# chenhuims/DistributedDeepLearningSpark

Hardware: AMD Instinct MI355X
Metric: images/sec (whole node) ResNet-50 ImageNet-shape at 1/2/4/8 MI355X (higher is better)
Workload: dtype bf16; 1 GPU; model=resnet50, global_batch=256, image=224, per_gpu_batch=256, parallelism=dp1, optimizer=sgd-momentum, buckets=4

## Files before the change

distributeddeeplearningspark_amd/csrc/include/ddl_ops.h:

```cpp
#pragma once
#include <hip/hip_runtime.h>
#include <stdint.h>

namespace ddl {

inline uint32_t drop_t8(double p) {
  if (!(p > 0.0)) return 0u;
  const double t = p * 256.0 + 0.5;
  return t < 1.0 ? 1u : (t >= 255.0 ? 255u : (uint32_t)t);
}
inline float drop_scale8(uint32_t t8) { return t8 ? (float)(256.0 / (256.0 - (double)t8)) : 1.f; }

constexpr int kBnShards = 32;
constexpr int kMaxPartials = 512;

int bn_partial_rows(long M, int C);
int splitk_finalize(float* ws, void* y, const float* bias, float* stats, long M, int C, int relu, int splits,
                    long slab_stride, hipStream_t s, long brows = 0,
                    long zbias = 0);
int bn_stats(const void* x, float* ws, long M, int C, hipStream_t s);
int bn_finalize(const float* ws, int S, long M, int C, const float* gamma, const float* beta, float eps,
                float momentum, float* running_mean, float* running_var, float* save_mean, float* save_invstd,
                float* scale, float* shift, hipStream_t s);
int bn_apply(const void* x, const float* scale, const float* shift, const void* resid, void* y, void* mask, long M,
             int C, int relu, hipStream_t s, const float* res_scale = nullptr, const float* res_shift = nullptr);
int bn_bwd_reduce(const void* dy, const void* x, const void* y, const float* scale, const float* shift,
                  const float* mean, float* ws, long M, int C, int mode, hipStream_t s);
int bn_bwd_finalize(const float* ws, int S, long M, int C, const float* gamma, const float* mean, const float* invstd,
                    float* dgamma, float* dbeta, float* coef, hipStream_t s);
int bn_bwd_dx(const void* dy, const void* x, const void* y, const float* scale, const float* shift,
              const float* coef, void* dx, void* dres, long M, int C, int mode, hipStream_t s,
              const void* x2 = nullptr, const float* mean2 = nullptr, float* ws2 = nullptr);

int bn_fold_sums(const void* w, long ldw, const float* P, const float* wsg, const float* mean, const float* wsy,
                 int rows, float* sums, float* s, int Co, int Ci, hipStream_t st);
int bn_fold_coef(const void* w, long ldw, const float* P, const float* S, const float* s, const float* coef, void* WA,
                 void* WAt, void* Gm, float* kv, float* dW, long lddw, int Co, int Ci, hipStream_t st);
int bn_fold_kv(const void* WA, const void* Gm, const float* sg, const float* s, long M, float* kv, int Co, int Ci,
               hipStream_t st);
int gram_colsum(const void* y2, long ld, long M, int Ci, float* S, float* s, int cus, hipStream_t st);
int bn_fold_fwd_stats(const void* w, long ldw, const float* S, const float* s, long M, float* ws, int Co, int Ci,
                      hipStream_t st);

bool pool3s2_bn_bwd_ok(int N, int H, int W, int C, int Ho, int Wo, int k = 3);
int pool3s2_bn_bwd(const void* dy, const uint8_t* am, const void* x, const float* scale, const float* shift,
                   const float* mean, const float* coef, float* ws, int S, void* dx, int N, int H, int W, int C, int Ho,
                   int Wo, hipStream_t s, int k = 3);

int maxpool_fwd(const void* x, void* y, uint8_t* argmax, int N, int H, int W, int C, int Ho, int Wo, int kh, int kw,
                int sh, int sw, int ph, int pw, hipStream_t s, const float* scale = nullptr, const float* shift = nullptr);
int maxpool_bwd(const void* dy, const uint8_t* argmax, void* dx, int N, int H, int W, int C, int Ho, int Wo, int kh,
                int kw, int sh, int sw, int ph, int pw, hipStream_t s);
int avgpool_global_fwd(const void* x, void* y, int N, int HW, int C, hipStream_t s);
int avgpool_global_bwd(const void* dy, void* dx, int N, int HW, int C, hipStream_t s);

int softmax_xent(const void* logits, int logits_bf16, const int64_t* labels, const float* target_probs,
                 float* loss_rows, void* dlogits, int B, int K, long ld, float grad_scale, float label_smoothing,
                 int ignore_index, hipStream_t s, const float* grad_scale_dev = nullptr, float* loss_out = nullptr,
                 float out_scale = 1.f, int zrows = 0);
int label_count_inv(const int64_t* labels, long n, int ignore_index, float* inv, hipStream_t s);
int rows_sum_scaled(const float* rows, long n, float scale, const float* dev, float* out, hipStream_t s);
int scale_bf16_dev(void* x, long n, const float* s_dev, hipStream_t s);
int mse_fwd_bwd(const float* pred, const float* target, long n, float* loss, float* grad, hipStream_t s);
int prob_xent(const float* p, const int64_t* labels, const float* target, float* loss_rows, float* dp, int B, int K,
              float eps, float scale, int ignore_index, hipStream_t s);
int mask_count_inv(const uint8_t* mask, long n, float* inv, hipStream_t s);
int temporal_xent(const float* logits, const int64_t* labels, const float* target_probs, const uint8_t* mask,
                  const float* inv_dev, float inv_host, float* loss_rows, float* dlogits, long R, int K, hipStream_t s);
int temporal_reg(const float* pred, const float* target, const uint8_t* mask, long R, int F, int mae, float* loss,
                 float* grad, hipStream_t s);

int cast_f32_bf16(const float* x, void* y, long n, hipStream_t s);
int cast_bf16_f32(const void* x, float* y, long n, hipStream_t s);
int sum_rows_bf16(const void* x, void* y, int R, long n, hipStream_t s);
int relu_bwd(const void* dy, const void* y, void* dx, long n, hipStream_t s);
// ... 224 lines not shown
```

distributeddeeplearningspark_amd/csrc/kernels/gemm_stream.hip:

```cpp
#include "ddl_gemm_kernel.h"

namespace ddl {
namespace gst {

constexpr int THREADS = 256;
constexpr int BM = 64;
constexpr int LDS_BUDGET = 80 * 1024;
typedef __attribute__((address_space(3))) void lds_t;

template <int WN, int K, bool CSM = false>
struct Cfg {
  static constexpr int NB = 4 * WN;
  static constexpr int RN = WN / 16;
  static constexpr int KS = K / 32;
  static constexpr int CPR = K / 8;
  static constexpr int TILE = BM * K * 2;
  static constexpr int D = TILE / 1024 / 4;
  static constexpr int OCPR = NB / 8;
  static constexpr int STAGE = BM * NB * 2;
  static constexpr int RPP = THREADS / OCPR;
  static constexpr int S = BM / RPP;
  static constexpr int SV = CSM ? 2 * S : S;
  static constexpr int NBUF_FIT = (LDS_BUDGET - STAGE) / TILE;
  static constexpr int NBUF = NBUF_FIT > 4 ? 4 : NBUF_FIT;
  static constexpr int LDS = NBUF * TILE + STAGE;
  static_assert(NBUF >= 2, "A ring needs two buffers");
  static_assert(D >= 1 && OCPR >= 8 && RPP >= 1 && BM % RPP == 0, "shape");
  static_assert((NBUF - 1) * (D + SV) <= 63, "vmcnt range");
  static_assert(4 * 2 * OCPR * 8 * 4 <= STAGE, "stats reduction fits in the staging buffer");
};

template <int CPR>
__device__ __forceinline__ int sw(int r) {
  if constexpr (CPR == 8) return (r >> 1) & 7;
  else return r & 15;
}

template <int N>
__device__ __forceinline__ void wait_vm() {
  __builtin_amdgcn_s_waitcnt((N & 15) | ((N >> 4) << 14) | 0x0F70);
}

template <class CF, int SV = CF::S>
__device__ __forceinline__ void wait_tile(int younger_store_tiles) {
  constexpr int base = (CF::NBUF - 1) * CF::D;
  switch (younger_store_tiles) {
    case 0: wait_vm<base>(); break;
    case 1: wait_vm<base + SV>(); break;
    case 2: wait_vm<base + 2 * SV>(); break;
    default: wait_vm<base + 3 * SV>(); break;
  }
}

template <class CF, bool DUAL = false>
__device__ __forceinline__ void stage_a(const bf16_t* __restrict__ A, long lda, int M, int m0, char* slot, int w,
                                        int lane, const bf16_t* __restrict__ A2 = nullptr, long lda2 = 0) {
#pragma unroll
  for (int i = 0; i < CF::D; ++i) {
    const int blk = i * 4 + w;
    const int u = blk * 64 + lane;
    const int r = u / CF::CPR, cp = u % CF::CPR;
    const int c = cp ^ sw<CF::CPR>(r);
    const int gr = min(m0 + r, M - 1);
    const bf16_t* src = A + (long)gr * lda + c * 8;
    if constexpr (DUAL) {
      if (c >= CF::CPR / 2) src = A2 + (long)gr * lda2 + (c - CF::CPR / 2) * 8;
    }
    const uint32_t dst = __builtin_amdgcn_readfirstlane((uint32_t) reinterpret_cast<uintptr_t>((lds_t*)(slot + blk * 1024)));
    asm volatile("s_mov_b32 m0, %1\n\tglobal_load_lds_dwordx4 %0, off" ::"v"(src), "s"(dst) : "memory", "m0");
  }
}

}

typedef __attribute__((ext_vector_type(2))) unsigned u32x2_t;
typedef __attribute__((ext_vector_type(4))) unsigned u32x4_t;
__device__ __forceinline__ u32x4_t ald128(const void* p) {
  u32x4_t v;
  asm volatile("global_load_dwordx4 %0, %1, off" : "=v"(v) : "v"(p) : "memory");
  return v;
}
__device__ __forceinline__ u32x2_t ald64(const void* p) {
  u32x2_t v;
  asm volatile("global_load_dwordx2 %0, %1, off" : "=v"(v) : "v"(p) : "memory");
  return v;
}
__device__ __forceinline__ unsigned ald32(const void* p) {
  unsigned v;
  asm volatile("global_load_dword %0, %1, off" : "=v"(v) : "v"(p) : "memory");
  return v;
}
__device__ __forceinline__ unsigned ald16(const void* p) {
  unsigned v;
  asm volatile("global_load_ushort %0, %1, off" : "=v"(v) : "v"(p) : "memory");
  return v;
}
__device__ __forceinline__ unsigned ald8(const void* p) {
  unsigned v;
  asm volatile("global_load_ubyte %0, %1, off" : "=v"(v) : "v"(p) : "memory");
  return v;
}
template <bool ASM> __device__ __forceinline__ u32x4_t sld128(const void* p) {
// ... 378 lines not shown
    (void)hipGetDevice(&dev);
    if (hipDeviceGetAttribute(&cus, hipDeviceAttributeMultiprocessorCount, dev) != hipSuccess || cus <= 0) cus = 256;
  }
  return cus;
}

template <int WN, int K, int BMODE>
int launch_ws(const GemmParams& p, hipStream_t s) {
  using CF = gst::Cfg<WN, K>;
  constexpr bool kRes = !(WN == 64 && K == 128);
  constexpr bool kBnr = CF::NB <= (K >= 256 ? 64 : 128);
  const int panels = p.N / CF::NB;
  const int mt = (p.M + gst::BM - 1) / gst::BM;
  const int gx = std::max(1, std::min(mt, 2 * num_cus() / std::max(1, panels)));
  if (p.colscale || p.relu_mask_out) {
    constexpr bool kCsm = BMODE == OP_KC && ((WN == 64 && K == 64) || (WN == 32 && K == 128) || (WN == 32 && K == 256));
    if constexpr (kCsm) {
      if (!p.colscale || !p.resid || p.bnr_x || p.bnr_premask || p.stats || p.rsub_h) return (int)hipErrorInvalidValue;
      hipLaunchKernelGGL((gemm_stream_kernel<WN, K, BMODE, true, 0, true>), dim3(gx, panels), dim3(gst::THREADS), 0, s, p);
    } else {
      return (int)hipErrorInvalidValue;
    }
  } else if (p.bnr_premask) {
    if constexpr (kBnr && kRes && BMODE == OP_RC) {
      if (!p.bnr_mask || p.bnr_scale) return (int)hipErrorInvalidValue;
      if (p.resid)
        hipLaunchKernelGGL((gemm_stream_kernel<WN, K, BMODE, true, 3>), dim3(gx, panels), dim3(gst::THREADS), 0, s, p);
      else
        hipLaunchKernelGGL((gemm_stream_kernel<WN, K, BMODE, false, 3>), dim3(gx, panels), dim3(gst::THREADS), 0, s, p);
    } else {
      return (int)hipErrorInvalidValue;
    }
  } else if (p.bnr_x && p.bnr_scale) {
    constexpr bool kRes2 = WN == 16 && K == 256 && BMODE == OP_RC;
    if constexpr (kBnr) {
      if (p.resid) {
        if constexpr (kRes2)
          hipLaunchKernelGGL((gemm_stream_kernel<WN, K, BMODE, true, 2>), dim3(gx, panels), dim3(gst::THREADS), 0, s, p);
        else
          return (int)hipErrorInvalidValue;
      } else {
        hipLaunchKernelGGL((gemm_stream_kernel<WN, K, BMODE, false, 2>), dim3(gx, panels), dim3(gst::THREADS), 0, s, p);
      }
    } else {
      return (int)hipErrorInvalidValue;
    }
  } else if (p.bnr_x) {
    if constexpr (kBnr && kRes) {
      if (p.resid)
        hipLaunchKernelGGL((gemm_stream_kernel<WN, K, BMODE, true, 1>), dim3(gx, panels), dim3(gst::THREADS), 0, s, p);
      else
        hipLaunchKernelGGL((gemm_stream_kernel<WN, K, BMODE, false, 1>), dim3(gx, panels), dim3(gst::THREADS), 0, s, p);
    } else if constexpr (kBnr) {
      if (p.resid) return (int)hipErrorInvalidValue;
      hipLaunchKernelGGL((gemm_stream_kernel<WN, K, BMODE, false, 1>), dim3(gx, panels), dim3(gst::THREADS), 0, s, p);
    } else {
      return (int)hipErrorInvalidValue;
    }
  } else if (p.resid) {
    if constexpr (kRes)
      hipLaunchKernelGGL((gemm_stream_kernel<WN, K, BMODE, true>), dim3(gx, panels), dim3(gst::THREADS), 0, s, p);
    else
      return (int)hipErrorInvalidValue;
  } else {
    hipLaunchKernelGGL((gemm_stream_kernel<WN, K, BMODE, false>), dim3(gx, panels), dim3(gst::THREADS), 0, s, p);
  }
  return (int)hipGetLastError();
// ... 73 lines not shown
```

distributeddeeplearningspark_amd/csrc/ops_bindings.cpp:

```cpp
#include <torch/extension.h>
#include <ATen/hip/impl/HIPStreamMasqueradingAsCUDA.h>
#include <ATen/DeviceGuard.h>

#include "ddl_ops.h"

namespace py = pybind11;
using namespace ddl;

namespace {

inline hipStream_t cur_stream() { return at::hip::getCurrentHIPStreamMasqueradingAsCUDA().stream(); }

#define CK(cond, ...) TORCH_CHECK(cond, __VA_ARGS__)
#define GPU(x) CK((x).is_cuda(), #x " must be a GPU tensor")
#define BF16(x) CK((x).scalar_type() == at::kBFloat16 && (x).is_contiguous(), #x " must be contiguous bf16")
#define F32(x) CK((x).scalar_type() == at::kFloat && (x).is_contiguous(), #x " must be contiguous fp32")
#define HIP_OK(expr)                                                                  \
  do {                                                                                \
    int _e = (expr);                                                                  \
    CK(_e == 0, "HIP launch failed: ", hipGetErrorString((hipError_t)_e)); \
  } while (0)

template <class T>
T* optr(const c10::optional<at::Tensor>& t) {
// ... 95 lines not shown
void bn_fold_sums_(const at::Tensor& w, const at::Tensor& P, const at::Tensor& wsg, const at::Tensor& mean,
                   c10::optional<at::Tensor> wsy, const at::Tensor& sums, const at::Tensor& s) {
  GPU(w); F32(P); F32(wsg); F32(mean); F32(sums); F32(s);
  CK(w.scalar_type() == at::kBFloat16 && w.dim() == 2 && w.stride(1) == 1, "bn_fold_sums: w [Co, Ci] bf16");
  const int64_t Co = w.size(0), Ci = w.size(1);
  CK(P.numel() == Co * Ci && wsg.numel() == (int64_t)kBnShards * 2 * Co && mean.numel() >= Co && sums.numel() == 2 * Co &&
         s.numel() == Ci,
     "bn_fold_sums: shapes");
  if (wsy) { F32(*wsy); CK(wsy->numel() % (2 * Ci) == 0 && wsy->numel() > 0, "bn_fold_sums: wsy [rows, 2, Ci]"); }
  at::DeviceGuard g(w.device());
  HIP_OK(bn_fold_sums(w.data_ptr(), w.stride(0), P.data_ptr<float>(), wsg.data_ptr<float>(), mean.data_ptr<float>(),
                      optr<const float>(wsy), wsy ? (int)(wsy->numel() / (2 * Ci)) : 0, sums.data_ptr<float>(),
                      s.data_ptr<float>(), (int)Co, (int)Ci, cur_stream()));
}

void gram_colsum_(const at::Tensor& y2, const at::Tensor& S, const at::Tensor& s) {
  GPU(y2); GPU(S); GPU(s); F32(S); F32(s);
  CK(y2.scalar_type() == at::kBFloat16 && y2.dim() == 2 && y2.stride(1) == 1 && y2.stride(0) % 8 == 0 &&
         ((uintptr_t)y2.data_ptr() % 16) == 0,
     "gram_colsum: y2 [M, Ci] bf16, 16-B aligned rows");
  const int64_t M = y2.size(0), Ci = y2.size(1);
  CK((Ci == 64 || Ci == 128 || Ci == 256) && M > 0 && y2.stride(0) >= Ci, "gram_colsum: Ci in {64, 128, 256}");
  CK(S.numel() == Ci * Ci && s.numel() == Ci && ((uintptr_t)S.data_ptr() % 16) == 0, "gram_colsum: S [Ci, Ci], s [Ci]");
  CK(S.device() == y2.device() && s.device() == y2.device(), "gram_colsum: y2, S and s on one device");
  at::DeviceGuard g(y2.device());
  static int cus_of[64] = {};
  const int dev = y2.device().index();
  int cus = dev >= 0 && dev < 64 ? cus_of[dev] : 0;
  if (!cus) {
    if (hipDeviceGetAttribute(&cus, hipDeviceAttributeMultiprocessorCount, dev) != hipSuccess || cus <= 0) cus = 256;
    if (dev >= 0 && dev < 64) cus_of[dev] = cus;
  }
  HIP_OK(gram_colsum(y2.data_ptr(), y2.stride(0), M, (int)Ci, S.data_ptr<float>(), s.data_ptr<float>(), cus, cur_stream()));
}

void bn_fold_fwd_stats_(const at::Tensor& w, const at::Tensor& S, const at::Tensor& s, int64_t M, const at::Tensor& ws) {
  GPU(w); GPU(S); GPU(s); GPU(ws); F32(S); F32(s); F32(ws);
  CK(S.device() == w.device() && s.device() == w.device() && ws.device() == w.device(),
     "bn_fold_fwd_stats: w, S, s and ws on one device");
  CK(w.scalar_type() == at::kBFloat16 && w.dim() == 2 && w.stride(1) == 1, "bn_fold_fwd_stats: w [Co, Ci] bf16");
  const int64_t Co = w.size(0), Ci = w.size(1);
  CK(Ci % 32 == 0 && Ci <= 256 && M > 0 && S.numel() == Ci * Ci && s.numel() == Ci && ws.numel() >= 2 * Co &&
         ((uintptr_t)S.data_ptr() % 16) == 0,
     "bn_fold_fwd_stats: Ci % 32 == 0, Ci <= 256, S [Ci, Ci], s [Ci], ws [>= 1, 2, Co]");
  at::DeviceGuard g(w.device());
  HIP_OK(bn_fold_fwd_stats(w.data_ptr(), w.stride(0), S.data_ptr<float>(), s.data_ptr<float>(), M, ws.data_ptr<float>(),
                           (int)Co, (int)Ci, cur_stream()));
}

void bn_fold_coef_(const at::Tensor& w, const at::Tensor& P, const at::Tensor& S, const at::Tensor& s,
                   const at::Tensor& coef, const at::Tensor& WA, const at::Tensor& WAt, const at::Tensor& Gm,
                   const at::Tensor& kv, const at::Tensor& dW) {
  GPU(w); F32(P); F32(S); F32(s); F32(coef); BF16(WA); BF16(WAt); BF16(Gm); F32(kv);
  CK(w.scalar_type() == at::kBFloat16 && w.dim() == 2 && w.stride(1) == 1, "bn_fold_coef: w [Co, Ci] bf16");
  const int64_t Co = w.size(0), Ci = w.size(1);
  CK(Co % 128 == 0 && Ci % 64 == 0, "bn_fold_coef: Co % 128, Ci % 64");
  CK(P.numel() == Co * Ci && S.numel() == Ci * Ci && s.numel() == Ci && coef.numel() >= 3 * Co && WA.numel() == Co * Ci &&
         WAt.numel() == Co * Ci && Gm.numel() == Ci * Ci && kv.numel() == Ci,
     "bn_fold_coef: shapes");
  CK(dW.is_cuda() && dW.scalar_type() == at::kFloat && dW.dim() == 2 && dW.size(0) == Co && dW.size(1) == Ci &&
         dW.stride(1) == 1 && dW.stride(0) >= Ci,
     "bn_fold_coef: dW [Co, Ci] fp32");
  at::DeviceGuard g(w.device());
  HIP_OK(bn_fold_coef(w.data_ptr(), w.stride(0), P.data_ptr<float>(), S.data_ptr<float>(), s.data_ptr<float>(),
                      coef.data_ptr<float>(), WA.data_ptr(), WAt.data_ptr(), Gm.data_ptr(), kv.data_ptr<float>(),
                      dW.data_ptr<float>(), dW.stride(0), (int)Co, (int)Ci, cur_stream()));
// ... 586 lines not shown
  OPT_CHECK(w, g);
  F32(acc);
  CK(acc.numel() == w.numel(), "rmsprop: state size");
  if (w16) BF16(*w16);
  at::DeviceGuard gd(w.device());
  HIP_OK(rmsprop_step(w.data_ptr<float>(), g.data_ptr<float>(), acc.data_ptr<float>(), optr<void>(w16), w.numel(),
                      (float)lr, (float)rho, (float)eps, (float)wd, (float)gscale, cur_stream()));
}
void sumsq_(const at::Tensor& x, const at::Tensor& out) {
  GPU(x); F32(x); F32(out);
  CK(x.numel() % 4 == 0, "sumsq: multiple of 4");
  at::DeviceGuard gd(x.device());
  HIP_OK(sumsq_f32(x.data_ptr<float>(), x.numel(), out.data_ptr<float>(), cur_stream()));
}

}

void register_ops(py::module& m) {
  m.attr("BN_SHARDS") = (int)kBnShards;
  m.def("bn_stats", &bn_stats_);
  m.def("splitk_finalize", &splitk_finalize_, py::arg("ws"), py::arg("y"), py::arg("C"), py::arg("bias"), py::arg("relu"),
        py::arg("stats"), py::arg("splits") = 0, py::arg("brows") = 0, py::arg("zbias") = 0);
  m.def("bn_partial_rows", &bn_partial_rows_);
  m.def("bn_finalize", &bn_finalize_);
  m.def("bn_apply", &bn_apply_, py::arg("x"), py::arg("scale"), py::arg("shift"), py::arg("resid"), py::arg("y"),
        py::arg("C"), py::arg("relu"), py::arg("mask") = py::none(), py::arg("res_scale") = py::none(),
        py::arg("res_shift") = py::none());
  m.def("bn_bwd_reduce", &bn_bwd_reduce_);
  m.def("bn_bwd_finalize", &bn_bwd_finalize_);
  m.def("bn_fold_sums", &bn_fold_sums_);
  m.def("bn_fold_coef", &bn_fold_coef_);
  m.def("bn_fold_kv", &bn_fold_kv_);
  m.def("gram_colsum", &gram_colsum_);
  m.def("bn_fold_fwd_stats", &bn_fold_fwd_stats_);
  m.def("bn_bwd_dx", &bn_bwd_dx_);
  m.def("bn_bwd_dx_red", &bn_bwd_dx_red_);
  m.def("pool3s2_bn_bwd", &pool3s2_bn_bwd_, py::arg("dy"), py::arg("am"), py::arg("x"), py::arg("scale"),
        py::arg("shift"), py::arg("mean"), py::arg("coef_or_ws"), py::arg("dx"), py::arg("k") = 3);
  m.def("pool3s2_bn_bwd_ok", [](int64_t N, int64_t H, int64_t W, int64_t C, int64_t Ho, int64_t Wo, int64_t k) {
    return pool3s2_bn_bwd_ok((int)N, (int)H, (int)W, (int)C, (int)Ho, (int)Wo, (int)k);
  });
  m.def("maxpool_fwd", &maxpool_fwd_, "NHWC max pool (byte argmax); optional fused BN affine + ReLU on load",
        py::arg("x"), py::arg("y"), py::arg("am"), py::arg("kh"), py::arg("kw"), py::arg("sh"), py::arg("sw"),
        py::arg("ph"), py::arg("pw"), py::arg("scale") = py::none(), py::arg("shift") = py::none());
  m.def("maxpool_bwd", &maxpool_bwd_);
  m.def("avgpool_fwd", &avgpool_fwd_);
  m.def("avgpool_bwd", &avgpool_bwd_);
  m.def("softmax_xent", &softmax_xent_, "fused softmax cross-entropy", py::arg("logits"), py::arg("labels"),
        py::arg("probs"), py::arg("loss_rows"), py::arg("dlogits"), py::arg("grad_scale"), py::arg("smoothing"),
        py::arg("ignore_index"), py::arg("grad_scale_dev") = py::none(), py::arg("loss_out") = py::none(),
        py::arg("out_scale") = 1.0, py::arg("zrows") = 0);
  m.def("label_count_inv", &label_count_inv_);
  m.def("rows_sum_scaled", &rows_sum_scaled_);
  m.def("pad_cols_bf16", &pad_cols_bf16_, "zero-padded copy of a row-strided bf16 view");
  m.def("zero_ranges", &zero_ranges_, "zero up to 8 contiguous device buffers in one launch", py::arg("buffers"));
  m.def("gather_bf16", &gather_bf16_, "out[i] = src[idx[i]] (0 where idx < 0)", py::arg("src"), py::arg("idx"),
        py::arg("out"), py::arg("src_extent"));
  m.def("scatter_add_f32", &scatter_add_f32_, "dst[idx[i]] += src[i] (idx injective, < 0 skipped)", py::arg("src"),
        py::arg("idx"), py::arg("dst"), py::arg("dst_extent"));
  m.def("scale_bf16_dev", &scale_bf16_dev_);
  m.def("cast_f32_bf16", &cast_f32_bf16_);
  m.def("sum_rows_bf16", &sum_rows_bf16_);
  m.def("cast_bf16_f32", &cast_bf16_f32_);
  m.def("relu_bwd", &relu_bwd_);
  m.def("add_bf16", &add_bf16_);
  m.def("bias_grad", &bias_grad_, py::arg("dy"), py::arg("db"), py::arg("N"), py::arg("accumulate"),
// ... 34 lines not shown
```

distributeddeeplearningspark_amd/ops/fused_blocks.py:

```python
from __future__ import annotations

import weakref

import torch

from . import conv as CV
from . import determinism as _det
from . import gemm as G
from . import zpad as ZP
from ._native import C
from .norm import new_stats_workspace, partials_workspace, pool_epoch
from .streams import on_grad_stream


class _ConvBNState:

    __slots__ = ("g", "yc", "y", "mean", "invstd", "scale", "shift", "mode", "mask", "pre_reduced", "fold", "gram",
                 "__weakref__")

    def __init__(self):
        self.pre_reduced = None
        self.fold = False
        self.gram = None

# ... 321 lines not shown
    ps = new_stats_workspace(-(-(Ci * Ci + Ci) // 64), dev).view(-1)
    S, s = ps[: Ci * Ci].view(Ci, Ci), ps[Ci * Ci : Ci * Ci + Ci]
    C().gram_colsum(xm, S, s)
    stats = new_stats_workspace(Co, dev)
    C().bn_fold_fwd_stats(conv.kernel.data.view(Co, Ci), S, s, M, stats)
    gamma = None if bn.gamma is None else bn.gamma.master
    beta = None if bn.beta is None else bn.beta.master
    rm, rv = bn._states["moving_mean"], bn._states["moving_variance"]
    st = _ConvBNState()
    st.g, st.yc, st.y, st.mask = g, None, None, None
    st.scale, st.shift, st.mean, st.invstd = torch.empty(4, Co, dtype=torch.float32, device=dev).unbind(0)
    C().bn_finalize(stats, M, Co, gamma, beta, bn.epsilon, 1.0 - bn.momentum, rm, rv, st.mean, st.invstd, st.scale,
                    st.shift)
    st.gram = (S, s, pool_epoch(dev))
    return st


def _fold_down_forward(block, x, y2, g3, gd):
    M, Co = g3.M, g3.Co
    if tuple(y2.shape) != (g3.N, g3.H, g3.W, g3.Ci):
        raise RuntimeError("folding projection block: conv2's output does not match conv3's geometry")
    y2 = y2.contiguous()
    s3 = _fold_fwd_stats(block.c3, y2.view(M, g3.Ci), g3)
    sd = _fold_fwd_stats(block.down, x.view(M, gd.Ci), gd)
    s3.mask = torch.empty(-(-M * Co // 32) * 4, dtype=torch.uint8, device=x.device)
    y = torch.empty((g3.N, g3.H, g3.W, Co), dtype=torch.bfloat16, device=x.device)
    G.linear_dual_fwd(y2.view(M, g3.Ci), block.c3.conv.kernel.data.view(Co, g3.Ci), s3.scale,
                      x.view(M, gd.Ci), block.down.conv.kernel.data.view(Co, gd.Ci), sd.scale,
                      shift1=s3.shift, shift2=sd.shift, relu=True, out=y.view(M, Co), relu_mask_out=s3.mask)
    s3.y, s3.mode, sd.mode = y, 3, 0
    return sd, s3


def fold_conv_bn_backward(w, gw, g2, y2, ws_g, mean, invstd, gamma, dgamma, dbeta, bnr2=None, out=None, gram=None,
                          need_dx=True, exact_colsum=False):
    M, Co = g2.shape
    Ci = y2.shape[1]
    dev = g2.device
    if gram is not None:
        S, s = gram
        P = new_stats_workspace(-(-(Co * Ci) // 64), dev).view(-1)[: Co * Ci].view(Co, Ci)
        G.linear_wgrad(g2, y2, P)
        wsy = None
    else:
        ps = new_stats_workspace(-(-(Co * Ci + Ci * Ci + Ci) // 64), dev).view(-1)
        P, S = ps[: Co * Ci].view(Co, Ci), ps[Co * Ci : Co * Ci + Ci * Ci].view(Ci, Ci)
        s = ps[Co * Ci + Ci * Ci : Co * Ci + Ci * Ci + Ci]
        G.linear_wgrad(g2, y2, P)
        G.linear_wgrad(y2, y2, S)
        wsy = partials_workspace(M, Ci, dev)
        C().bn_stats(y2, wsy, Ci)
    f32 = torch.empty(5 * Co + Ci, dtype=torch.float32, device=dev)
    sums, coef, kv = f32[: 2 * Co], f32[2 * Co : 5 * Co], f32[5 * Co :]
    C().bn_fold_sums(w, P, ws_g, mean, wsy, sums, s)
    C().bn_bwd_finalize(sums, M, Co, gamma, mean, invstd, dgamma, dbeta, coef)
    b16 = torch.empty(2 * Co * Ci + Ci * Ci, dtype=torch.bfloat16, device=dev)
    WA, WAt, Gm = b16[: Co * Ci].view(Co, Ci), b16[Co * Ci : 2 * Co * Ci].view(Ci, Co), b16[2 * Co * Ci :].view(Ci, Ci)
    C().bn_fold_coef(w, P, S, s, coef, WA, WAt, Gm, kv, gw)
    if not need_dx:
        return None, sums.view(2, Co)
    if exact_colsum:
        C().bn_fold_kv(WA, Gm, sums[:Co], s, M, kv)
    r = G.linear_fwd(y2, Gm, bias=kv)
    if out is None:
        out = torch.empty((M, Ci), dtype=torch.bfloat16, device=dev)
    G.linear_dgrad(g2, WA, out=out, resid=r, bnr=bnr2, wt=WAt)
    return out, sums.view(2, Co)


def _fold_bn3_backward(unit, s3, s2, g, ws_g, bnr2):
    return _fold_unit_backward(unit, s3, s2.y, g, ws_g, bnr2)


def _fold_unit_backward(unit, st, xin, g, ws_g, bnr2, need_dx=True, exact_colsum=False):
    conv, bn = unit.conv, unit.bn
    geo = st.g
    M, Co, Ci = geo.M, geo.Co, geo.Ci
    dx = torch.empty((geo.N, geo.H, geo.W, Ci), dtype=torch.bfloat16, device=g.device) if need_dx else None
    gram = None
    if st.gram is not None and st.gram[2] == pool_epoch(g.device):
        gram = st.gram[:2]
    fold_conv_bn_backward(conv.kernel.data.view(Co, Ci), conv.kernel.grad.view(Co, Ci), g.view(M, Co), xin.view(M, Ci),
                          ws_g, st.mean, st.invstd, bn.gamma.master, bn.gamma.grad,
                          None if bn.beta is None else bn.beta.grad, bnr2=bnr2,
                          out=None if dx is None else dx.view(M, Ci), gram=gram, need_dx=need_dx,
                          exact_colsum=exact_colsum)
    if bn.grad_hook is not None:
        bn.grad_hook()
    if conv.grad_hook is not None:
        conv.grad_hook()
    return dx


def _same_tensor(a, b) -> bool:
    return (a.data_ptr() == b.data_ptr() and a.shape == b.shape and a.stride() == b.stride()
            and a._version == b._version)


# ... 292 lines not shown
```

distributeddeeplearningspark_amd/ops/gemm.py:

```python
from __future__ import annotations

import math

import torch

from . import determinism as _det
from ._native import C

KC, RC, KC_GATHER, RC_GATHER, RC_TAPS, KC_GATHER8, RC_GATHER8 = 0, 1, 2, 3, 4, 5, 6
EPI_BF16, EPI_F32, EPI_F32_ATOMIC = 0, 1, 2
TILE256 = 4
TILE_STREAM = 5
TILE_CONV3 = 6
_TILES = {0: (128, 128), 1: (128, 64), 2: (64, 128), 3: (64, 64), TILE256: (256, 256), TILE_STREAM: (64, 256),
          TILE_CONV3: (224, 128)}
_ONE_PER_CU = (TILE256,)
_CU = 256
import os as _os

_USE256 = "auto"


_USE_STREAM = "1"
_TILE_FILL = 2.0
# ... 237 lines not shown
            r = gemm(dy, w, ws, M, K, N, KC, RC, dy.stride(0), w.stride(0), K, EPI_F32, tile=3,
                     k_split=math.ceil(N / splits / 64) * 64, defer_slabs=True)
        if isinstance(r, tuple):
            C().splitk_finalize(r[0], out, K, None, False, stats, r[1])
        else:
            C().splitk_finalize(ws, out, K, None, False, stats)
        return out
    if M >= _WT_MIN_M and not use_stream(M, K, N, KC, RC, EPI_BF16, dy.stride(0), out.stride(0), aux=gelu_pre,
                                         relu=act, resid=resid, ldr=ldr):
        wt = transpose(w) if wt is None else wt
        fb = _bnr_plain_ok(bnr, stats, resid, gelu_pre, K)
        gemm(dy, wt, out, M, K, N, KC, KC, dy.stride(0), wt.stride(0), out.stride(0), EPI_BF16, resid=resid,
             ldr=ldr, relu=act, aux=gelu_pre, stats=stats, resid_mask=resid_mask, rsub=rsub, bnr=bnr if fb else None)
        if fb:
            bnr["done"] = True
        return out
    if (bnr is not None and stats is None
            and ("scale" not in bnr or (resid is None and rsub is None) or (rsub is None and (K, N) == (64, 256)))
            and use_stream(M, K, N, KC, RC, EPI_BF16, dy.stride(0), out.stride(0), aux=gelu_pre, relu=act,
                           resid=resid, ldr=ldr)):
        gemm(dy, w, out, M, K, N, KC, RC, dy.stride(0), w.stride(0), out.stride(0), EPI_BF16, resid=resid, ldr=ldr,
             relu=act, aux=gelu_pre, resid_mask=resid_mask, tile=TILE_STREAM, bnr=bnr, rsub=rsub)
        bnr["done"] = True
        return out
    fb = _bnr_plain_ok(bnr, stats, resid, gelu_pre, K) and not use_stream(
        M, K, N, KC, RC, EPI_BF16, dy.stride(0), out.stride(0), aux=gelu_pre, relu=act, resid=resid, ldr=ldr)
    gemm(dy, w, out, M, K, N, KC, RC, dy.stride(0), w.stride(0), out.stride(0), EPI_BF16, resid=resid,
         ldr=ldr, relu=act, aux=gelu_pre, stats=stats, resid_mask=resid_mask, rsub=rsub, bnr=bnr if fb else None)
    if fb:
        bnr["done"] = True
    return out


def _bnr_plain_ok(bnr, stats, resid, gelu_pre, ncols) -> bool:
    return (bnr is not None and stats is None and gelu_pre is None and ncols % 8 == 0
            and (bnr["x"].is_contiguous() if bnr.get("x") is not None else bool(bnr.get("premask")))
            and (resid is None or (resid.stride(0) % 4 == 0 and resid.data_ptr() % 8 == 0)))


def transpose(w):
    R, Cc = w.shape
    if w.stride(1) != 1 or R % 8 or Cc % 8 or w.stride(0) % 8:
        return w.t().contiguous()
    if w.is_contiguous():
        from . import derived

        return derived.taps_transpose(w, (0,), (Cc, R))
    out = torch.empty((Cc, R), dtype=w.dtype, device=w.device)
    C().transpose_bf16(w, out)
    return out


def linear_wgrad(dy, x2, gw):
    M, N = dy.shape
    K = x2.shape[1]
    rounds = None if (big_wgrad(N, K, M) and _SPLITK_SLABS_MODE == "auto") else _LINEAR_WGRAD_ROUNDS
    return gemm(dy, x2, gw, N, K, M, RC, RC, dy.stride(0), x2.stride(0), gw.stride(0), EPI_F32, beta=1.0,
                split_rounds=rounds)


def matmul(a, b, trans_a=False, trans_b=False, out=None, alpha=1.0):
    M = a.shape[1] if trans_a else a.shape[0]
    K = a.shape[0] if trans_a else a.shape[1]
    N = b.shape[0] if trans_b else b.shape[1]
    if out is None:
        out = torch.empty((M, N), dtype=torch.bfloat16, device=a.device)
# ... 4 lines not shown
```

Before: 13410 images/sec.

## Fuse fold-BN backward wgrad and dgrad into a single pass over g and y2

Adds a HIP kernel for the Co=256/Ci=64 folded conv+BN backward. It streams g and y2 through LDS once, computing the P = g^T·y2 weight-gradient product and the t = g·(gamma*invstd*W) data-gradient product together. A second GEMM pass then adds y2·Gm+kv using t as the residual, replacing the separate linear_wgrad, linear_fwd and linear_dgrad launches. This cuts re-reads of the large g activation, but adds a bf16 intermediate t, atomics into P, and one-off weight scaling per block.

```diff
diff --git a/distributeddeeplearningspark_amd/csrc/include/ddl_gemm_stream.h b/distributeddeeplearningspark_amd/csrc/include/ddl_gemm_stream.h
--- /dev/null
+++ b/distributeddeeplearningspark_amd/csrc/include/ddl_gemm_stream.h
@@ -0,0 +1,28 @@
+#pragma once
+#include "ddl_common.h"
+
+namespace ddl {
+namespace gst {
+
+constexpr int THREADS = 256;
+constexpr int BM = 64;
+typedef __attribute__((address_space(3))) void lds_t;
+
+template <int CPR>
+__device__ __forceinline__ int sw(int r) {
+  if constexpr (CPR == 8) return (r >> 1) & 7;
+  else return r & 15;
+}
+
+template <int N>
+__device__ __forceinline__ void wait_vm() {
+  __builtin_amdgcn_s_waitcnt((N & 15) | ((N >> 4) << 14) | 0x0F70);
+}
+
+__device__ __forceinline__ void dma_1k(const void* src, char* dst_block) {
+  const uint32_t dst = __builtin_amdgcn_readfirstlane((uint32_t) reinterpret_cast<uintptr_t>((lds_t*)dst_block));
+  asm volatile("s_mov_b32 m0, %1\n\tglobal_load_lds_dwordx4 %0, off" ::"v"(src), "s"(dst) : "memory", "m0");
+}
+
+}
+}
diff --git a/distributeddeeplearningspark_amd/csrc/include/ddl_ops.h b/distributeddeeplearningspark_amd/csrc/include/ddl_ops.h
--- a/distributeddeeplearningspark_amd/csrc/include/ddl_ops.h
+++ b/distributeddeeplearningspark_amd/csrc/include/ddl_ops.h
@@ -41,6 +41,9 @@
 int gram_colsum(const void* y2, long ld, long M, int Ci, float* S, float* s, int cus, hipStream_t st);
 int bn_fold_fwd_stats(const void* w, long ldw, const float* S, const float* s, long M, float* ws, int Co, int Ci,
                       hipStream_t st);
+int fold_bwd_pass1(const void* g, long ldg, const void* y2, long ldy, const void* w, long ldw, const float* gamma,
+                   const float* invstd, long M, int Co, int Ci, float* P, void* t, long ldt, void* wa_out,
+                   int workgroups, hipStream_t st);
 
 bool pool3s2_bn_bwd_ok(int N, int H, int W, int C, int Ho, int Wo, int k = 3);
 int pool3s2_bn_bwd(const void* dy, const uint8_t* am, const void* x, const float* scale, const float* shift,
diff --git a/distributeddeeplearningspark_amd/csrc/kernels/fold_bwd.hip b/distributeddeeplearningspark_amd/csrc/kernels/fold_bwd.hip
--- /dev/null
+++ b/distributeddeeplearningspark_amd/csrc/kernels/fold_bwd.hip
@@ -0,0 +1,238 @@
+#include "ddl_gemm_stream.h"
+#include "ddl_ops.h"
+
+namespace ddl {
+namespace fbw {
+
+using gst::BM;
+using gst::sw;
+using gst::wait_vm;
+
+constexpr int THREADS = 256;
+constexpr int CO = 256, CI = 64;
+constexpr int GROW = CO * 2, YROW = CI * 2;
+constexpr int GT = BM * GROW, YT = BM * YROW;
+constexpr int GCPR = CO / 8, YCPR = CI / 8;
+constexpr int NBUF = 3;
+constexpr int CHAIN = 8;
+constexpr int MIN_TILES = 16;
+constexpr int STAGE = BM * CI * 2;
+constexpr int S = STAGE / 16 / THREADS;
+
+struct Cfg {
+  static constexpr int SLOT = GT + YT;
+  static constexpr int D = SLOT / 1024 / 4;
+  static constexpr int LDS = NBUF * SLOT + STAGE;
+  static_assert((NBUF - 1) * (D + S) <= 63, "vmcnt range");
+  static_assert(LDS <= 160 * 1024, "LDS");
+};
+
+__device__ __forceinline__ void stage(const bf16_t* __restrict__ g, long ldg, const bf16_t* __restrict__ y, long ldy,
+                                      int M, int m0, char* slot, int w, int lane) {
+#pragma unroll
+  for (int i = 0; i < Cfg::D; ++i) {
+    const int blk = i * 4 + w;
+    const bf16_t* src;
+    if (i < GT / 4096) {
+      const int u = blk * 64 + lane;
+      const int r = u / GCPR, c = (u % GCPR) ^ sw<GCPR>(r);
+      src = g + (long)min(m0 + r, M - 1) * ldg + c * 8;
+    } else {
+      const int u = (blk - GT / 1024) * 64 + lane;
+      const int r = u / YCPR, c = (u % YCPR) ^ sw<YCPR>(r);
+      src = y + (long)min(m0 + r, M - 1) * ldy + c * 8;
+    }
+    gst::dma_1k(src, slot + blk * 1024);
+  }
+}
+
+template <int CPR>
+__device__ __forceinline__ bf16x8 tr_frag(const char* lds, int kk, int c0, int lane) {
+  const int g = lane >> 4, li = lane & 15, q = li >> 2, p = li & 3;
+  const int k1 = kk * 32 + 8 * g + q, k2 = k1 + 4;
+  const int col = c0 + 4 * p;
+  const int ch = col >> 3, within = (col & 7) * 2;
+  const int o1 = k1 * (CPR * 16) + ((ch ^ sw<CPR>(k1)) << 4) + within;
+  const int o2 = k2 * (CPR * 16) + ((ch ^ sw<CPR>(k2)) << 4) + within;
+  const s16x4 lo = __builtin_amdgcn_ds_read_tr16_b64_v4i16((DDL_LDS s16x4*)(lds + o1));
+  const s16x4 hi = __builtin_amdgcn_ds_read_tr16_b64_v4i16((DDL_LDS s16x4*)(lds + o2));
+  const s16x8 r = {lo[0], lo[1], lo[2], lo[3], hi[0], hi[1], hi[2], hi[3]};
+  return __builtin_bit_cast(bf16x8, r);
+}
+
+__device__ __forceinline__ void wait_tile(int younger_store_tiles) {
+  constexpr int base = (NBUF - 1) * Cfg::D;
+  switch (younger_store_tiles) {
+    case 0: wait_vm<base>(); break;
+    case 1: wait_vm<base + S>(); break;
+    default: wait_vm<base + 2 * S>(); break;
+  }
+}
+
+}
+
+__global__ __launch_bounds__(fbw::THREADS, 1) void fold_bwd_pass1_kernel(
+    const bf16_t* __restrict__ g, long ldg, const bf16_t* __restrict__ y2, long ldy, const bf16_t* __restrict__ wgt,
+    long ldw, const float* __restrict__ gamma, const float* __restrict__ invstd, int M, float* __restrict__ P,
+    bf16_t* __restrict__ t, long ldt, bf16_t* __restrict__ wa_out) {
+  using namespace fbw;
+  using CF = Cfg;
+  __shared__ __attribute__((aligned(16))) char smem[CF::LDS];
+  char* const stg = smem + NBUF * CF::SLOT;
+  const int lane = threadIdx.x & 63, w = threadIdx.x >> 6;
+  const int mh = w >> 1, nh = w & 1;
+  const int mt = (M + BM - 1) / BM;
+  const int nloc = ((int)blockIdx.x < mt) ? (mt - 1 - (int)blockIdx.x) / (int)gridDim.x + 1 : 0;
+
+  bf16x8 wa[2][CO / 32];
+#pragma unroll
+  for (int rn = 0; rn < 2; ++rn)
+#pragma unroll
+    for (int ks = 0; ks < CO / 32; ++ks) {
+      const int ci = 32 * nh + 16 * rn + (lane & 15);
+      s16x8 v;
+#pragma unroll
+      for (int j = 0; j < 8; ++j) {
+        const int co = 32 * ks + 8 * (lane >> 4) + j;
+        const float a = gamma[co] * invstd[co];
+        const bf16_t b = f2bf(a * bf2f(wgt[(long)co * ldw + ci]));
+        v[j] = (short)b;
+      }
+      wa[rn][ks] = __builtin_bit_cast(bf16x8, v);
+    }
+  if (wa_out && blockIdx.x == 0) {
+    for (int u = threadIdx.x; u < CO * CI; u += THREADS) {
+      const int co = u / CI, ci = u % CI;
+      const float a = gamma[co] * invstd[co];
+      wa_out[u] = f2bf(a * bf2f(wgt[(long)co * ldw + ci]));
+    }
+  }
+  wait_vm<0>();
+  auto tile_m0 = [&](int i) { return min((int)blockIdx.x + i * (int)gridDim.x, mt - 1) * BM; };
+
+#pragma unroll
+  for (int s = 0; s < NBUF - 1; ++s) stage(g, ldg, y2, ldy, M, tile_m0(s), smem + s * CF::SLOT, w, lane);
+
+  f32x4 acc[4][4], tot[4][4];
+#pragma unroll
+  for (int cb = 0; cb < 4; ++cb)
+#pragma unroll
+    for (int nb = 0; nb < 4; ++nb)
+      acc[cb][nb] = tot[cb][nb] = f32x4{0.f, 0.f, 0.f, 0.f};
+  auto fold_chain = [&]() {
+#pragma unroll
+    for (int cb = 0; cb < 4; ++cb)
+#pragma unroll
+      for (int nb = 0; nb < 4; ++nb) {
+        tot[cb][nb] += acc[cb][nb];
+        acc[cb][nb] = f32x4{0.f, 0.f, 0.f, 0.f};
+      }
+  };
+  const int oc = threadIdx.x % YCPR, orow = threadIdx.x / YCPR;
+  constexpr int RPP = THREADS / YCPR;
+
+  for (int i = 0; i < nloc; ++i) {
+    const int m0 = tile_m0(i);
+    const int ahead = i + NBUF - 1;
+    stage(g, ldg, y2, ldy, M, tile_m0(ahead), smem + (ahead % NBUF) * CF::SLOT, w, lane);
+    wait_tile(min(i, NBUF - 1));
+    __builtin_amdgcn_s_barrier();
+    char* const gbuf = smem + (i % NBUF) * CF::SLOT;
+    char* const ybuf = gbuf + GT;
+    if (m0 + BM > M) {
+      const int rz = M - m0;
+      for (int u = threadIdx.x; u < (BM - rz) * YCPR; u += THREADS)
+        *reinterpret_cast<uint4*>(ybuf + rz * YROW + u * 16) = make_uint4(0u, 0u, 0u, 0u);
+      __builtin_amdgcn_s_waitcnt(0xC07F);
+      __builtin_amdgcn_s_barrier();
+    }
+
+    f32x4 tacc[2][2];
+#pragma unroll
+    for (int mb = 0; mb < 2; ++mb)
+#pragma unroll
+      for (int rn = 0; rn < 2; ++rn) tacc[mb][rn] = f32x4{0.f, 0.f, 0.f, 0.f};
+#pragma unroll
+    for (int ks = 0; ks < CO / 32; ++ks)
+#pragma unroll
+      for (int mb = 0; mb < 2; ++mb) {
+        const int r = 32 * mh + 16 * mb + (lane & 15);
+        const int c = 4 * ks + (lane >> 4);
+        const bf16x8 a = *reinterpret_cast<const bf16x8*>(gbuf + r * GROW + ((c ^ sw<GCPR>(r)) << 4));
+#pragma unroll
+        for (int rn = 0; rn < 2; ++rn) tacc[mb][rn] = mfma16x16x32(wa[rn][ks], a, tacc[mb][rn]);
+      }
+
+    __builtin_amdgcn_sched_barrier(0);
+    {
+      bf16x8 gf[4][2];
+#pragma unroll
+      for (int cb = 0; cb < 4; ++cb)
+#pragma unroll
+        for (int kk = 0; kk < 2; ++kk) gf[cb][kk] = tr_frag<GCPR>(gbuf, kk, 64 * w + 16 * cb, lane);
+#pragma unroll
+      for (int nb = 0; nb < 4; ++nb) {
+        const bf16x8 y0 = tr_frag<YCPR>(ybuf, 0, 16 * nb, lane);
+        const bf16x8 y1 = tr_frag<YCPR>(ybuf, 1, 16 * nb, lane);
+#pragma unroll
+        for (int cb = 0; cb < 4; ++cb) {
+          acc[cb][nb] = mfma16x16x32(gf[cb][0], y0, acc[cb][nb]);
+          acc[cb][nb] = mfma16x16x32(gf[cb][1], y1, acc[cb][nb]);
+        }
+        __builtin_amdgcn_sched_barrier(0);
+      }
+    }
+    if (i % CHAIN == CHAIN - 1) fold_chain();
+
+#pragma unroll
+    for (int mb = 0; mb < 2; ++mb) {
+      const int r = 32 * mh + 16 * mb + (lane & 15);
+#pragma unroll
+      for (int rn = 0; rn < 2; ++rn) {
+        const int nl = 32 * nh + 16 * rn + 4 * (lane >> 4);
+        *reinterpret_cast<uint2*>(stg + r * YROW + (((nl >> 3) ^ sw<YCPR>(r)) << 4) + (nl & 7) * 2) =
+            make_uint2(pack_bf16x2(tacc[mb][rn][0], tacc[mb][rn][1]), pack_bf16x2(tacc[mb][rn][2], tacc[mb][rn][3]));
+      }
+    }
+    __builtin_amdgcn_s_waitcnt(0xC07F);
+    __builtin_amdgcn_s_barrier();
+
+#pragma unroll
+    for (int ps = 0; ps < S; ++ps) {
+      const int r = orow + ps * RPP;
+      const uint4 v = *reinterpret_cast<const uint4*>(stg + r * YROW + ((oc ^ sw<YCPR>(r)) << 4));
+      if (m0 + r < M) *reinterpret_cast<uint4*>(t + (long)(m0 + r) * ldt + oc * 8) = v;
+    }
+  }
+  wait_vm<0>();
+
+  fold_chain();
+  if (nloc > 0) {
+#pragma unroll
+    for (int cb = 0; cb < 4; ++cb)
+#pragma unroll
+      for (int nb = 0; nb < 4; ++nb)
+#pragma unroll
+        for (int e = 0; e < 4; ++e) {
+          const long idx = (long)(64 * w + 16 * cb + 4 * (lane >> 4) + e) * CI + 16 * nb + (lane & 15);
+          atomicAdd(P + idx, tot[cb][nb][e]);
+        }
+  }
+}
+
+int fold_bwd_pass1(const void* g, long ldg, const void* y2, long ldy, const void* w, long ldw, const float* gamma,
+                   const float* invstd, long M, int Co, int Ci, float* P, void* t, long ldt, void* wa_out,
+                   int workgroups, hipStream_t st) {
+  auto al16 = [](const void* q) { return (uintptr_t)q % 16 == 0; };
+  if (Co != fbw::CO || Ci != fbw::CI || M <= 0 || M >= (1L << 30) || workgroups <= 0 || !g || !y2 || !w || !gamma ||
+      !invstd || !P || !t || ldg % 8 || ldy % 8 || ldt % 8 || ldg < Co || ldy < Ci || ldt < Ci || ldw < Ci || !al16(g) ||
+      !al16(y2) || !al16(t))
+    return (int)hipErrorInvalidValue;
+  const int mt = (int)((M + gst::BM - 1) / gst::BM);
+  const dim3 grid((unsigned)std::max(1, std::min((mt + fbw::MIN_TILES - 1) / fbw::MIN_TILES, workgroups)));
+  hipLaunchKernelGGL(fold_bwd_pass1_kernel, grid, dim3(fbw::THREADS), 0, st, (const bf16_t*)g, ldg, (const bf16_t*)y2,
+                     ldy, (const bf16_t*)w, ldw, gamma, invstd, (int)M, P, (bf16_t*)t, ldt, (bf16_t*)wa_out);
+  return (int)hipGetLastError();
+}
+
+}
diff --git a/distributeddeeplearningspark_amd/csrc/kernels/gemm_stream.hip b/distributeddeeplearningspark_amd/csrc/kernels/gemm_stream.hip
--- a/distributeddeeplearningspark_amd/csrc/kernels/gemm_stream.hip
+++ b/distributeddeeplearningspark_amd/csrc/kernels/gemm_stream.hip
@@ -1,12 +1,10 @@
 #include "ddl_gemm_kernel.h"
+#include "ddl_gemm_stream.h"
 
 namespace ddl {
 namespace gst {
 
-constexpr int THREADS = 256;
-constexpr int BM = 64;
 constexpr int LDS_BUDGET = 80 * 1024;
-typedef __attribute__((address_space(3))) void lds_t;
 
 template <int WN, int K, bool CSM = false>
 struct Cfg {
@@ -30,17 +28,6 @@
   static_assert(4 * 2 * OCPR * 8 * 4 <= STAGE, "stats reduction fits in the staging buffer");
 };
 
-template <int CPR>
-__device__ __forceinline__ int sw(int r) {
-  if constexpr (CPR == 8) return (r >> 1) & 7;
-  else return r & 15;
-}
-
-template <int N>
-__device__ __forceinline__ void wait_vm() {
-  __builtin_amdgcn_s_waitcnt((N & 15) | ((N >> 4) << 14) | 0x0F70);
-}
-
 template <class CF, int SV = CF::S>
 __device__ __forceinline__ void wait_tile(int younger_store_tiles) {
   constexpr int base = (CF::NBUF - 1) * CF::D;
@@ -66,8 +53,7 @@
     if constexpr (DUAL) {
       if (c >= CF::CPR / 2) src = A2 + (long)gr * lda2 + (c - CF::CPR / 2) * 8;
     }
-    const uint32_t dst = __builtin_amdgcn_readfirstlane((uint32_t) reinterpret_cast<uintptr_t>((lds_t*)(slot + blk * 1024)));
-    asm volatile("s_mov_b32 m0, %1\n\tglobal_load_lds_dwordx4 %0, off" ::"v"(src), "s"(dst) : "memory", "m0");
+    dma_1k(src, slot + blk * 1024);
   }
 }
 
@@ -512,7 +498,7 @@
       return (int)hipErrorInvalidValue;
     }
   } else if (p.bnr_x && p.bnr_scale) {
-    constexpr bool kRes2 = WN == 16 && K == 256 && BMODE == OP_RC;
+    constexpr bool kRes2 = WN == 16 && (K == 256 || K == 64) && BMODE == OP_RC;
     if constexpr (kBnr) {
       if (p.resid) {
         if constexpr (kRes2)
diff --git a/distributeddeeplearningspark_amd/csrc/ops_bindings.cpp b/distributeddeeplearningspark_amd/csrc/ops_bindings.cpp
--- a/distributeddeeplearningspark_amd/csrc/ops_bindings.cpp
+++ b/distributeddeeplearningspark_amd/csrc/ops_bindings.cpp
@@ -151,6 +151,44 @@
     if (dev >= 0 && dev < 64) cus_of[dev] = cus;
   }
   HIP_OK(gram_colsum(y2.data_ptr(), y2.stride(0), M, (int)Ci, S.data_ptr<float>(), s.data_ptr<float>(), cus, cur_stream()));
+}
+
+bool fold_bwd_pass1_ok_(int64_t Co, int64_t Ci) { return Co == 256 && Ci == 64; }
+
+void fold_bwd_pass1_(const at::Tensor& g, const at::Tensor& y2, const at::Tensor& w, const at::Tensor& gamma,
+                     const at::Tensor& invstd, const at::Tensor& P, const at::Tensor& t,
+                     c10::optional<at::Tensor> wa_out, int64_t max_workgroups) {
+  GPU(g); GPU(y2); GPU(w); GPU(gamma); GPU(invstd); GPU(P); GPU(t);
+  BF16(g); BF16(y2); BF16(w); BF16(t); F32(gamma); F32(invstd); F32(P);
+  auto rows_ok = [](const at::Tensor& a) {
+    return a.dim() == 2 && a.stride(1) == 1 && a.stride(0) % 8 == 0 && a.stride(0) >= a.size(1) &&
+           ((uintptr_t)a.data_ptr() % 16) == 0;
+  };
+  CK(rows_ok(g) && rows_ok(y2) && rows_ok(t), "fold_bwd_pass1: g, y2, t [M, C] bf16 with 16-B aligned rows");
+  const int64_t M = g.size(0), Co = g.size(1), Ci = y2.size(1);
+  CK(fold_bwd_pass1_ok_(Co, Ci) && M > 0 && y2.size(0) == M && t.size(0) == M && t.size(1) == Ci,
+     "fold_bwd_pass1: (Co, Ci) = (256, 64), y2 and t [M, Ci]");
+  CK(w.dim() == 2 && w.size(0) == Co && w.size(1) == Ci && w.stride(1) == 1 && w.stride(0) >= Ci, "fold_bwd_pass1: w [Co, Ci]");
+  CK(gamma.numel() >= Co && invstd.numel() >= Co && gamma.is_contiguous() && invstd.is_contiguous(),
+     "fold_bwd_pass1: gamma, invstd [Co]");
+  CK(P.numel() == Co * Ci && P.is_contiguous(), "fold_bwd_pass1: P [Co, Ci]");
+  const auto dev = g.device();
+  CK(y2.device() == dev && w.device() == dev && gamma.device() == dev && invstd.device() == dev && P.device() == dev &&
+         t.device() == dev,
+     "fold_bwd_pass1: all tensors on one device");
+  if (wa_out) {
+    GPU(*wa_out); BF16(*wa_out);
+    CK(wa_out->numel() == Co * Ci && wa_out->is_contiguous() && wa_out->device() == dev, "fold_bwd_pass1: wa_out [Co, Ci]");
+  }
+  CK(max_workgroups >= 0, "fold_bwd_pass1: max_workgroups >= 0");
+  at::DeviceGuard guard(dev);
+  int wgs = (int)std::min<int64_t>(max_workgroups, 1 << 20);
+  if (!wgs) {
+    if (hipDeviceGetAttribute(&wgs, hipDeviceAttributeMultiprocessorCount, dev.index()) != hipSuccess || wgs <= 0) wgs = 256;
+  }
+  HIP_OK(fold_bwd_pass1(g.data_ptr(), g.stride(0), y2.data_ptr(), y2.stride(0), w.data_ptr(), w.stride(0),
+                        gamma.data_ptr<float>(), invstd.data_ptr<float>(), M, (int)Co, (int)Ci, P.data_ptr<float>(),
+                        t.data_ptr(), t.stride(0), wa_out ? wa_out->data_ptr() : nullptr, wgs, cur_stream()));
 }
 
 void bn_fold_fwd_stats_(const at::Tensor& w, const at::Tensor& S, const at::Tensor& s, int64_t M, const at::Tensor& ws) {
@@ -803,6 +841,9 @@
   m.def("bn_fold_coef", &bn_fold_coef_);
   m.def("bn_fold_kv", &bn_fold_kv_);
   m.def("gram_colsum", &gram_colsum_);
+  m.def("fold_bwd_pass1_ok", &fold_bwd_pass1_ok_);
+  m.def("fold_bwd_pass1", &fold_bwd_pass1_, py::arg("g"), py::arg("y2"), py::arg("w"), py::arg("gamma"),
+        py::arg("invstd"), py::arg("P"), py::arg("t"), py::arg("wa_out") = py::none(), py::arg("max_workgroups") = 0);
   m.def("bn_fold_fwd_stats", &bn_fold_fwd_stats_);
   m.def("bn_bwd_dx", &bn_bwd_dx_);
   m.def("bn_bwd_dx_red", &bn_bwd_dx_red_);
diff --git a/distributeddeeplearningspark_amd/ops/fused_blocks.py b/distributeddeeplearningspark_amd/ops/fused_blocks.py
--- a/distributeddeeplearningspark_amd/ops/fused_blocks.py
+++ b/distributeddeeplearningspark_amd/ops/fused_blocks.py
@@ -377,21 +377,44 @@
     return sd, s3
 
 
+_FOLD_ONEPASS = True
+
+
+def _onepass_ok(w, g2, y2, gamma, invstd) -> bool:
+    def rows(a):
+        return a.dtype == torch.bfloat16 and a.stride(1) == 1 and a.stride(0) % 8 == 0 and a.data_ptr() % 16 == 0
+
+    return (_FOLD_ONEPASS and g2.is_cuda and C().fold_bwd_pass1_ok(g2.shape[1], y2.shape[1]) and rows(g2) and rows(y2)
+            and w.dtype == torch.bfloat16 and w.stride(1) == 1 and gamma.dtype == torch.float32
+            and invstd.dtype == torch.float32 and gamma.is_contiguous() and invstd.is_contiguous())
+
+
 def fold_conv_bn_backward(w, gw, g2, y2, ws_g, mean, invstd, gamma, dgamma, dbeta, bnr2=None, out=None, gram=None,
                           need_dx=True, exact_colsum=False):
     M, Co = g2.shape
     Ci = y2.shape[1]
     dev = g2.device
+    onepass = need_dx and not exact_colsum and _onepass_ok(w, g2, y2, gamma, invstd)
+    t = None
+
+    def p_product(P):
+        if onepass:
+            nonlocal t
+            t = torch.empty((M, Ci), dtype=torch.bfloat16, device=dev)
+            C().fold_bwd_pass1(g2, y2, w, gamma, invstd, P, t)
+        else:
+            G.linear_wgrad(g2, y2, P)
+
     if gram is not None:
         S, s = gram
         P = new_stats_workspace(-(-(Co * Ci) // 64), dev).view(-1)[: Co * Ci].view(Co, Ci)
-        G.linear_wgrad(g2, y2, P)
+        p_product(P)
         wsy = None
     else:
         ps = new_stats_workspace(-(-(Co * Ci + Ci * Ci + Ci) // 64), dev).view(-1)
         P, S = ps[: Co * Ci].view(Co, Ci), ps[Co * Ci : Co * Ci + Ci * Ci].view(Ci, Ci)
         s = ps[Co * Ci + Ci * Ci : Co * Ci + Ci * Ci + Ci]
-        G.linear_wgrad(g2, y2, P)
+        p_product(P)
         G.linear_wgrad(y2, y2, S)
         wsy = partials_workspace(M, Ci, dev)
         C().bn_stats(y2, wsy, Ci)
@@ -406,9 +429,12 @@
         return None, sums.view(2, Co)
     if exact_colsum:
         C().bn_fold_kv(WA, Gm, sums[:Co], s, M, kv)
-    r = G.linear_fwd(y2, Gm, bias=kv)
     if out is None:
         out = torch.empty((M, Ci), dtype=torch.bfloat16, device=dev)
+    if onepass:
+        G.fold_pass2(y2, Gm, kv, t, out, bnr=bnr2)
+        return out, sums.view(2, Co)
+    r = G.linear_fwd(y2, Gm, bias=kv)
     G.linear_dgrad(g2, WA, out=out, resid=r, bnr=bnr2, wt=WAt)
     return out, sums.view(2, Co)
 
diff --git a/distributeddeeplearningspark_amd/ops/gemm.py b/distributeddeeplearningspark_amd/ops/gemm.py
--- a/distributeddeeplearningspark_amd/ops/gemm.py
+++ b/distributeddeeplearningspark_amd/ops/gemm.py
@@ -293,6 +293,15 @@
     return out
 
 
+def fold_pass2(y2, gm, kv, t, out, bnr=None):
+    M, K = y2.shape
+    gemm(y2, gm, out, M, K, K, KC, RC, y2.stride(0), gm.stride(0), out.stride(0), EPI_BF16, bias=kv, resid=t,
+         ldr=t.stride(0), tile=TILE_STREAM, bnr=bnr)
+    if bnr is not None:
+        bnr["done"] = True
+    return out
+
+
 def _bnr_plain_ok(bnr, stats, resid, gelu_pre, ncols) -> bool:
     return (bnr is not None and stats is None and gelu_pre is None and ncols % 8 == 0
             and (bnr["x"].is_contiguous() if bnr.get("x") is not None else bool(bnr.get("premask")))
```

Result: no change. 13500 images/sec (median of 6 runs) (+0.7%).
